# whcorkran/mamba-TTS-project

Hardware: AMD Instinct MI355X
Metric: audio tokens/sec (teacher-forced fwd+bwd) per GPU; decode_step p50 latency (higher is better)
Workload: dtype bf16; 1 GPU; C2: MambaTTSDecoder 12L d_model=1024 fwd+bwd+clip+Adam, B=8/GPU T_audio=2048 T_text=128; model=MambaTTSDecoder-12L-d1024, global_batch=8, seq_len=2048, parallelism=dp1

## Files before the change

### mamba-tts-project_amd/mtts/csrc/skinny.hip

```cpp
#include "common.h"

namespace mtts {
namespace {

typedef short s16x8 __attribute__((ext_vector_type(8)));
typedef __bf16 bf16x8 __attribute__((ext_vector_type(8)));
typedef float f32x4 __attribute__((ext_vector_type(4)));

__device__ __forceinline__ f32x4 mfma16(const uint4& x, const uint4& y, f32x4 c) {
  return __builtin_amdgcn_mfma_f32_16x16x32_bf16(__builtin_bit_cast(bf16x8, x), __builtin_bit_cast(bf16x8, y), c, 0, 0,
                                                 0);
}

struct SkinnyP {
  const bf16_t* a;
  const bf16_t* b;
  void* c;
  int64_t lda, ldb, ldc;
  int m, n, k;
  int c_f32;
  float beta;
};

__device__ __forceinline__ void store4(const SkinnyP& p, int row, int col, f32x4 v) {
  if (row >= p.m || col >= p.n) return;
  if (p.c_f32) {
    float* cp = (float*)p.c + (int64_t)row * p.ldc + col;
    if (p.beta != 0.f) v += p.beta * *(const f32x4*)cp;
    *(f32x4*)cp = v;
  } else {
    bf16_t* cp = (bf16_t*)p.c + (int64_t)row * p.ldc + col;
    if (p.beta != 0.f) {
      const uint2 o = *(const uint2*)cp;
      v[0] += p.beta * __uint_as_float(o.x << 16);
      v[1] += p.beta * __uint_as_float(o.x & 0xffff0000u);
      v[2] += p.beta * __uint_as_float(o.y << 16);
      v[3] += p.beta * __uint_as_float(o.y & 0xffff0000u);
    }
    *(uint2*)cp = make_uint2((uint32_t)f2bf(v[0]) | ((uint32_t)f2bf(v[1]) << 16),
                             (uint32_t)f2bf(v[2]) | ((uint32_t)f2bf(v[3]) << 16));
  }
}

template <int MB, int NB>
__global__ __launch_bounds__(256) void skinny_n_kernel(SkinnyP p) {
  constexpr int RB = MB * 16;
  constexpr int PA = 4;
  __shared__ __attribute__((aligned(16))) f32x4 red[2][MB * NB][64];
  const int lane = threadIdx.x & 63, wave = threadIdx.x >> 6;
  const int row0 = blockIdx.x * RB;
  const int li = lane & 15, kq = (lane >> 4) * 8;
  const bf16_t* ap[MB];
  const bf16_t* bp[NB];
#pragma unroll
  for (int i = 0; i < MB; ++i) ap[i] = p.a + (int64_t)min(row0 + i * 16 + li, p.m - 1) * p.lda + kq + wave * 32;
#pragma unroll
  for (int j = 0; j < NB; ++j) bp[j] = p.b + (int64_t)min(j * 16 + li, p.n - 1) * p.ldb + kq + wave * 32;
  f32x4 acc[MB][NB];
#pragma unroll
  for (int i = 0; i < MB; ++i)
#pragma unroll
    for (int j = 0; j < NB; ++j) acc[i][j] = f32x4{0.f, 0.f, 0.f, 0.f};
  const int ni = (p.k / 32 - wave + 3) / 4;
  uint4 fa[PA][MB], fb[2][NB];
  auto load_a = [&](int i, int st) __attribute__((always_inline)) {
#pragma unroll
    for (int r = 0; r < MB; ++r) fa[st][r] = *(const uint4*)(ap[r] + i * 128);
  };
  auto load_b = [&](int i, int st) __attribute__((always_inline)) {
#pragma unroll
    for (int j = 0; j < NB; ++j) fb[st][j] = *(const uint4*)(bp[j] + i * 128);
  };
#pragma unroll
  for (int j = 0; j < PA; ++j)
    if (j < ni) load_a(j, j);
  if (ni > 0) load_b(0, 0);
  for (int i0 = 0; i0 < ni; i0 += PA) {
#pragma unroll
    for (int j = 0; j < PA; ++j) {
      const int i = i0 + j;
      if (i < ni) {
        if (i + 1 < ni) load_b(i + 1, (j + 1) & 1);
#pragma unroll
        for (int r = 0; r < MB; ++r)
#pragma unroll
          for (int c = 0; c < NB; ++c) acc[r][c] = mfma16(fb[j & 1][c], fa[j][r], acc[r][c]);
        if (i + PA < ni) load_a(i + PA, j);
      }
    }
  }
  if (wave >= 2) {
#pragma unroll
    for (int i = 0; i < MB; ++i)
#pragma unroll
      for (int j = 0; j < NB; ++j) red[wave - 2][i * NB + j][lane] = acc[i][j];
  }
  block_sync();
  if (wave < 2) {
#pragma unroll
    for (int i = 0; i < MB; ++i)
#pragma unroll
      for (int j = 0; j < NB; ++j) acc[i][j] += red[wave][i * NB + j][lane];
  }
  block_sync();
  if (wave == 1) {
#pragma unroll
    for (int i = 0; i < MB; ++i)
#pragma unroll
      for (int j = 0; j < NB; ++j) red[0][i * NB + j][lane] = acc[i][j];
  }
  block_sync();
  if (wave == 0) {
#pragma unroll
    for (int i = 0; i < MB; ++i)
#pragma unroll
      for (int j = 0; j < NB; ++j) store4(p, row0 + i * 16 + li, j * 16 + (lane >> 4) * 4, acc[i][j] + red[0][i * NB + j][lane]);
  }
}

template <int KS>
__global__ __launch_bounds__(256) void small_k_kernel(SkinnyP p) {
  const int lane = threadIdx.x & 63, wave = threadIdx.x >> 6;
  const int row0 = blockIdx.y * 64;
  const int col0 = blockIdx.x * 256 + wave * 64;
  if (col0 >= p.n) return;
  const int li = lane & 15, kq = (lane >> 4) * 8;
  const int g = lane >> 4;
  const int cw_off = (g & 1) * 16 + 8 * (g >> 1);
  uint4 old16[4][2];
  f32x4 old32[4][4];
  if (p.beta != 0.f) {
#pragma unroll
    for (int i = 0; i < 4; ++i) {
      const int row = row0 + i * 16 + li;
      if (p.c_f32) {
#pragma unroll
        for (int j = 0; j < 4; ++j) {
          const int col = col0 + j * 16 + 4 * g;
          old32[i][j] = (row < p.m && col < p.n) ? *(const f32x4*)((const float*)p.c + (int64_t)row * p.ldc + col)
                                                 : f32x4{0.f, 0.f, 0.f, 0.f};
        }
      } else {
#pragma unroll
        for (int q = 0; q < 2; ++q) {
          const int cw = col0 + q * 32 + cw_off;
          old16[i][q] = (row < p.m && cw < p.n) ? *(const uint4*)((const bf16_t*)p.c + (int64_t)row * p.ldc + cw)
                                                : make_uint4(0, 0, 0, 0);
        }
      }
    }
  }
  uint4 fa[4][KS], fb[4][KS];
#pragma unroll
  for (int i = 0; i < 4; ++i) {
    const bf16_t* ap = p.a + (int64_t)min(row0 + i * 16 + li, p.m - 1) * p.lda + kq;
#pragma unroll
    for (int s = 0; s < KS; ++s) fa[i][s] = *(const uint4*)(ap + s * 32);
  }
#pragma unroll
  for (int j = 0; j < 4; ++j) {
    const bf16_t* bp = p.b + (int64_t)min(col0 + j * 16 + li, p.n - 1) * p.ldb + kq;
#pragma unroll
    for (int s = 0; s < KS; ++s) fb[j][s] = *(const uint4*)(bp + s * 32);
  }
  f32x4 acc[4][4];
#pragma unroll
  for (int i = 0; i < 4; ++i)
#pragma unroll
    for (int j = 0; j < 4; ++j) {
      acc[i][j] = f32x4{0.f, 0.f, 0.f, 0.f};
#pragma unroll
      for (int s = 0; s < KS; ++s) acc[i][j] = mfma16(fb[j][s], fa[i][s], acc[i][j]);
    }
  if (p.c_f32) {
#pragma unroll
    for (int i = 0; i < 4; ++i) {
      const int row = row0 + i * 16 + li;
#pragma unroll
      for (int j = 0; j < 4; ++j) {
        const int col = col0 + j * 16 + 4 * g;
        f32x4 v = acc[i][j];
        if (p.beta != 0.f) v += p.beta * old32[i][j];
        if (row < p.m && col < p.n) *(f32x4*)((float*)p.c + (int64_t)row * p.ldc + col) = v;
      }
    }
    return;
  }
#pragma unroll
  for (int i = 0; i < 4; ++i) {
    const int row = row0 + i * 16 + li;
#pragma unroll
    for (int q = 0; q < 2; ++q) {
      float v8[8];
#pragma unroll
      for (int e = 0; e < 4; ++e) {
        const auto r = __builtin_amdgcn_permlane16_swap(__float_as_uint(acc[i][2 * q][e]),
                                                        __float_as_uint(acc[i][2 * q + 1][e]), false, false);
        v8[e] = __uint_as_float(r[0]);
        v8[4 + e] = __uint_as_float(r[1]);
      }
      if (p.beta != 0.f) {
        const uint32_t ow[4] = {old16[i][q].x, old16[i][q].y, old16[i][q].z, old16[i][q].w};
#pragma unroll
        for (int e = 0; e < 4; ++e) {
          v8[2 * e] += p.beta * __uint_as_float(ow[e] << 16);
          v8[2 * e + 1] += p.beta * __uint_as_float(ow[e] & 0xffff0000u);
        }
      }
      uint32_t w[4];
#pragma unroll
      for (int e = 0; e < 4; ++e) w[e] = (uint32_t)f2bf(v8[2 * e]) | ((uint32_t)f2bf(v8[2 * e + 1]) << 16);
      const int cw = col0 + q * 32 + cw_off;
      if (row < p.m && cw < p.n) *(uint4*)((bf16_t*)p.c + (int64_t)row * p.ldc + cw) = make_uint4(w[0], w[1], w[2], w[3]);
    }
  }
}

constexpr int kTnRows = 64;
__device__ __forceinline__ int tn_off(int row, int ch) {
  return 256 * row + 16 * (ch ^ (((row & 3) << 2) | ((row >> 2) & 3)));
}
typedef short s16x4 __attribute__((ext_vector_type(4)));
typedef __attribute__((address_space(3))) s16x4 lds_s16x4;
__device__ __forceinline__ uint4 tn_frag(const char* img, int cb, int ks, int lane) {
  const int g = lane >> 4, q = (lane >> 2) & 3, pp = lane & 3;
  s16x4 r[2];
#pragma unroll
  for (int h = 0; h < 2; ++h) {
    const int row = ks * 32 + 8 * g + 4 * h + q;
    const int off = tn_off(row, cb * 2 + (pp >> 1)) + 8 * (pp & 1);
    r[h] = __builtin_amdgcn_ds_read_tr16_b64_v4i16((lds_s16x4*)(img + off));
  }
  s16x8 v{r[0][0], r[0][1], r[0][2], r[0][3], r[1][0], r[1][1], r[1][2], r[1][3]};
  return __builtin_bit_cast(uint4, v);
}

struct TnP {
  const bf16_t* a;
  const bf16_t* b;
  float* slab;
  int64_t lda, ldb;
  int m, n, k, kc;
};

template <int NB, bool TRANS>
__global__ __launch_bounds__(512) void tn_skinny_kernel(TnP p) {
  __shared__ __attribute__((aligned(16))) char sa[2][kTnRows * 256];
  __shared__ __attribute__((aligned(16))) char sb[2][kTnRows * 256];
  const int tid = threadIdx.x, lane = tid & 63, wave = tid >> 6;
  const int c0 = blockIdx.x * 128;
  const int k0 = blockIdx.y * p.kc, k1 = min(p.k, k0 + p.kc);
  const int ntile = (k1 - k0 + kTnRows - 1) / kTnRows;
  const int ch = tid & 15, r0 = tid >> 4;
  const bool bok = ch * 8 < p.n;
  uint4 ra[2], rb[2];
  auto load = [&](int t) __attribute__((always_inline)) {
#pragma unroll
    for (int s = 0; s < 2; ++s) {
      const int row = k0 + t * kTnRows + r0 + 32 * s;
      const bool ok = row < k1;
      const int rr = ok ? row : k0;
      ra[s] = *(const uint4*)(p.a + (int64_t)rr * p.lda + c0 + ch * 8);
      rb[s] = *(const uint4*)(p.b + (int64_t)rr * p.ldb + (bok ? ch * 8 : 0));
      if (!ok) ra[s] = make_uint4(0, 0, 0, 0);
      if (!ok || !bok) rb[s] = make_uint4(0, 0, 0, 0);
    }
  };
  auto store = [&](int buf) __attribute__((always_inline)) {
#pragma unroll
    for (int s = 0; s < 2; ++s) {
      *(uint4*)(sa[buf] + tn_off(r0 + 32 * s, ch)) = ra[s];
      *(uint4*)(sb[buf] + tn_off(r0 + 32 * s, ch)) = rb[s];
    }
  };
  f32x4 acc[NB];
#pragma unroll
  for (int j = 0; j < NB; ++j) acc[j] = f32x4{0.f, 0.f, 0.f, 0.f};
  if (ntile > 0) {
    load(0);
    store(0);
  }
  block_sync();
  for (int t = 0; t < ntile; ++t) {
    const int buf = t & 1;
    if (t + 1 < ntile) load(t + 1);
#pragma unroll
    for (int ks = 0; ks < 2; ++ks) {
      const uint4 fa = tn_frag(sa[buf], wave, ks, lane);
#pragma unroll
      for (int j = 0; j < NB; ++j) {
        const uint4 fb = tn_frag(sb[buf], j, ks, lane);
        acc[j] = TRANS ? mfma16(fa, fb, acc[j]) : mfma16(fb, fa, acc[j]);
      }
    }
    if (t + 1 < ntile) store(buf ^ 1);
    block_sync();
  }
  float* sl = p.slab + (int64_t)blockIdx.y * p.m * p.n;
  const int li = lane & 15, g4 = (lane >> 4) * 4;
#pragma unroll
  for (int j = 0; j < NB; ++j) {
    if constexpr (TRANS) {
      const int nn = j * 16 + li;
      if (nn < p.n) *(f32x4*)(sl + (int64_t)nn * p.m + c0 + wave * 16 + g4) = acc[j];
    } else {
      const int nn = j * 16 + g4;
      if (nn < p.n) *(f32x4*)(sl + (int64_t)(c0 + wave * 16 + li) * p.n + nn) = acc[j];
    }
  }
}

template <int MB>
void launch_skinny_n(const SkinnyP& p, hipStream_t st) {
  const int nb = (p.n + 15) / 16;
  const dim3 grid((p.m + MB * 16 - 1) / (MB * 16));
  switch (nb) {
#define SK_(N) case N: hipLaunchKernelGGL((skinny_n_kernel<MB, N>), grid, dim3(256), 0, st, p); break;
    SK_(1) SK_(2) SK_(3) SK_(4) SK_(5) SK_(6) SK_(7) SK_(8)
#undef SK_
  }
}

}
}

using namespace mtts;

static int tn_chunk(int k) { return k >= 8192 ? 512 : 256; }

extern "C" int64_t mtts_gemm_skinny_workspace(const MttsSkinnyArgs* a) {
  if (!a || a->mode != MTTS_SKINNY_TN || a->k <= 0) return 0;
  const int kc = tn_chunk(a->k);
  return (int64_t)((a->k + kc - 1) / kc) * a->m * a->n * 4 + 256;
}

static int skinny_tn(const MttsSkinnyArgs* a, hipStream_t st) {
  MTTS_CHECK(a->m % 128 == 0 && a->n <= 128 && a->n % 8 == 0,
             "gemm_skinny TN: needs m %% 128 == 0 and n <= 128, n %% 8 == 0 (m=%d n=%d)", a->m, a->n);
  MTTS_CHECK(a->c_dtype == MTTS_F32 && a->beta == 0.f, "gemm_skinny TN: fp32 output, beta = 0");
  MTTS_CHECK(a->workspace, "gemm_skinny TN: workspace required (mtts_gemm_skinny_workspace)");
  MTTS_CHECK(a->ldc == (a->trans_c ? a->m : a->n), "gemm_skinny TN: C must be contiguous (ldc = %d)",
             a->trans_c ? a->m : a->n);
  MTTS_CHECK(a->lda >= a->m && a->ldb >= a->n, "gemm_skinny TN: leading dimension too small");
  TnP p;
  p.a = (const bf16_t*)a->a; p.b = (const bf16_t*)a->b; p.slab = (float*)a->workspace;
  p.lda = a->lda; p.ldb = a->ldb; p.m = a->m; p.n = a->n; p.k = a->k; p.kc = tn_chunk(a->k);
  const int chunks = (a->k + p.kc - 1) / p.kc;
  const dim3 grid(a->m / 128, chunks);
  const int nb = (a->n + 15) / 16;
#define TN_(N)                                                                                        \
  case N:                                                                                             \
    if (a->trans_c) hipLaunchKernelGGL((tn_skinny_kernel<N, true>), grid, dim3(512), 0, st, p);      \
    else hipLaunchKernelGGL((tn_skinny_kernel<N, false>), grid, dim3(512), 0, st, p);                \
    break;
  switch (nb) { TN_(1) TN_(2) TN_(3) TN_(4) TN_(5) TN_(6) TN_(7) TN_(8) }
#undef TN_
  MTTS_LAUNCH_CHECK("gemm_skinny TN");
  const int ncols = a->m * a->n;
  colsum(p.slab, chunks, chunks, ncols, ncols, (float*)a->c, 0, st);
  MTTS_LAUNCH_CHECK("gemm_skinny TN chunk sum");
  return MTTS_OK;
}

extern "C" int mtts_gemm_skinny(const MttsSkinnyArgs* a, void* stream) {
  MTTS_CHECK(a && a->a && a->b && a->c, "gemm_skinny: null pointer");
  MTTS_CHECK(a->mode == MTTS_SKINNY_N || a->mode == MTTS_SKINNY_SMALL_K || a->mode == MTTS_SKINNY_TN,
             "gemm_skinny: bad mode %d", a->mode);
  MTTS_CHECK(a->m > 0 && a->n > 0 && a->k > 0, "gemm_skinny: m=%d n=%d k=%d must be positive", a->m, a->n, a->k);
  if (a->mode == MTTS_SKINNY_TN) {
    MTTS_CHECK(((uintptr_t)a->a | (uintptr_t)a->b | (uintptr_t)a->c) % 16 == 0 && a->lda % 8 == 0 && a->ldb % 8 == 0,
               "gemm_skinny TN: A / B / C must be 16-byte aligned with row strides a multiple of 8 elements");
    return skinny_tn(a, (hipStream_t)stream);
  }
  MTTS_CHECK(a->k % 32 == 0, "gemm_skinny: k=%d must be a multiple of 32", a->k);
  MTTS_CHECK(a->n % 4 == 0, "gemm_skinny: n=%d must be a multiple of 4", a->n);
  MTTS_CHECK(a->mode != MTTS_SKINNY_N || a->n <= 128, "gemm_skinny: SKINNY_N needs n <= 128 (n=%d)", a->n);
  MTTS_CHECK(a->mode != MTTS_SKINNY_SMALL_K || a->k <= 128, "gemm_skinny: SMALL_K needs k <= 128 (k=%d)", a->k);
  MTTS_CHECK(((uintptr_t)a->a | (uintptr_t)a->b) % 16 == 0 && a->lda % 8 == 0 && a->ldb % 8 == 0,
             "gemm_skinny: A / B must be 16-byte aligned with row strides a multiple of 8 elements");
  MTTS_CHECK(a->lda >= a->k && a->ldb >= a->k && a->ldc >= a->n, "gemm_skinny: leading dimension too small");
  MTTS_CHECK(a->c_dtype == MTTS_F32 || a->c_dtype == MTTS_BF16, "gemm_skinny: bad c_dtype");
  const int ces = a->c_dtype == MTTS_F32 ? 4 : 2;
  MTTS_CHECK((uintptr_t)a->c % (4 * ces) == 0 && a->ldc % 4 == 0,
             "gemm_skinny: C must be %d-byte aligned with ldc a multiple of 4", 4 * ces);
  MTTS_CHECK(a->mode != MTTS_SKINNY_SMALL_K || ces == 4 ||
                 (a->n % 8 == 0 && a->ldc % 8 == 0 && (uintptr_t)a->c % 16 == 0),
             "gemm_skinny: SMALL_K with bf16 C needs n %% 8 == 0, ldc %% 8 == 0 and a 16-byte aligned C "
             "(n=%d ldc=%d)", a->n, a->ldc);
  SkinnyP p;
  p.a = (const bf16_t*)a->a; p.b = (const bf16_t*)a->b; p.c = a->c;
  p.lda = a->lda; p.ldb = a->ldb; p.ldc = a->ldc;
  p.m = a->m; p.n = a->n; p.k = a->k;
  p.c_f32 = a->c_dtype == MTTS_F32;
  p.beta = a->beta;
  hipStream_t st = (hipStream_t)stream;
  if (a->mode == MTTS_SKINNY_N) {
    launch_skinny_n<4>(p, st);
  } else {
    const dim3 grid((a->n + 255) / 256, (a->m + 63) / 64);
    switch (a->k / 32) {
      case 1: hipLaunchKernelGGL((small_k_kernel<1>), grid, dim3(256), 0, st, p); break;
      case 2: hipLaunchKernelGGL((small_k_kernel<2>), grid, dim3(256), 0, st, p); break;
      case 3: hipLaunchKernelGGL((small_k_kernel<3>), grid, dim3(256), 0, st, p); break;
      default: hipLaunchKernelGGL((small_k_kernel<4>), grid, dim3(256), 0, st, p); break;
    }
  }
  MTTS_LAUNCH_CHECK("gemm_skinny");
  return MTTS_OK;
}
```

Baseline: 515,300 tokens/s.

## Restructure skinny GEMM kernels to stage tiles through swizzled LDS

The skinny-N kernel changes from per-wave K-splitting with an LDS reduction to one where each wave owns 16 rows. A and B tiles are cooperatively loaded into a double-buffered, XOR-swizzled LDS ring with register prefetch, and the output goes through LDS staging so stores are coalesced row-wise. The small-K kernel now stages A in LDS once per block instead of every wave reloading it from global memory. It also transposes accumulators through LDS for coalesced stores and sets a launch-bounds occupancy hint. This removes the cross-wave reduction and the redundant global loads, at the cost of a block barrier per K-tile and extra LDS traffic.

```diff
diff --git a/mamba-tts-project_amd/mtts/csrc/skinny.hip b/mamba-tts-project_amd/mtts/csrc/skinny.hip
--- a/mamba-tts-project_amd/mtts/csrc/skinny.hip
+++ b/mamba-tts-project_amd/mtts/csrc/skinny.hip
@@ -22,8 +22,7 @@
   float beta;
 };
 
-__device__ __forceinline__ void store4(const SkinnyP& p, int row, int col, f32x4 v) {
-  if (row >= p.m || col >= p.n) return;
+__device__ __forceinline__ void store_piece4(const SkinnyP& p, int row, int col, f32x4 v) {
   if (p.c_f32) {
     float* cp = (float*)p.c + (int64_t)row * p.ldc + col;
     if (p.beta != 0.f) v += p.beta * *(const f32x4*)cp;
@@ -42,177 +41,190 @@
   }
 }
 
-template <int MB, int NB>
-__global__ __launch_bounds__(256) void skinny_n_kernel(SkinnyP p) {
-  constexpr int RB = MB * 16;
-  constexpr int PA = 4;
-  __shared__ __attribute__((aligned(16))) f32x4 red[2][MB * NB][64];
-  const int lane = threadIdx.x & 63, wave = threadIdx.x >> 6;
-  const int row0 = blockIdx.x * RB;
-  const int li = lane & 15, kq = (lane >> 4) * 8;
-  const bf16_t* ap[MB];
-  const bf16_t* bp[NB];
-#pragma unroll
-  for (int i = 0; i < MB; ++i) ap[i] = p.a + (int64_t)min(row0 + i * 16 + li, p.m - 1) * p.lda + kq + wave * 32;
-#pragma unroll
-  for (int j = 0; j < NB; ++j) bp[j] = p.b + (int64_t)min(j * 16 + li, p.n - 1) * p.ldb + kq + wave * 32;
-  f32x4 acc[MB][NB];
-#pragma unroll
-  for (int i = 0; i < MB; ++i)
-#pragma unroll
-    for (int j = 0; j < NB; ++j) acc[i][j] = f32x4{0.f, 0.f, 0.f, 0.f};
-  const int ni = (p.k / 32 - wave + 3) / 4;
-  uint4 fa[PA][MB], fb[2][NB];
-  auto load_a = [&](int i, int st) __attribute__((always_inline)) {
-#pragma unroll
-    for (int r = 0; r < MB; ++r) fa[st][r] = *(const uint4*)(ap[r] + i * 128);
+__device__ __forceinline__ int kt_off(int row, int ch) { return row * 128 + ((ch ^ ((row >> 1) & 7)) << 4); }
+
+constexpr int kSkPF = 4;
+static_assert(kSkPF % 2 == 0, "kSkPF must be even");
+constexpr int kSkNW = 4;
+constexpr int kSkRB = 16 * kSkNW;
+constexpr int kSkRP = 8 * kSkNW;
+
+template <int NB>
+__global__ __launch_bounds__(64 * kSkNW) void skinny_n_kernel(SkinnyP p) {
+  constexpr int WR = NB * 16;
+  constexpr int WCH = (WR + kSkRP - 1) / kSkRP;
+  constexpr int A_BYTES = kSkRB * 128, SLOT = A_BYTES + WR * 128;
+  constexpr int CP = WR + 4;
+  static_assert(2 * SLOT >= kSkNW * 16 * CP * 4, "C staging fits the ring");
+  __shared__ __attribute__((aligned(16))) char lds[2 * SLOT];
+  const int tid = threadIdx.x, lane = tid & 63, wave = tid >> 6;
+  const int row0 = blockIdx.x * kSkRB;
+  const int ch = tid & 7, lr = (tid >> 3) & (kSkRP - 1);
+  const int li = lane & 15, g = lane >> 4;
+  const bf16_t* ap[2];
+  const bf16_t* bp[WCH];
+#pragma unroll
+  for (int s = 0; s < 2; ++s) ap[s] = p.a + (int64_t)min(row0 + lr + kSkRP * s, p.m - 1) * p.lda + ch * 8;
+#pragma unroll
+  for (int i = 0; i < WCH; ++i) bp[i] = p.b + (int64_t)min(lr + kSkRP * i, p.n - 1) * p.ldb + ch * 8;
+  f32x4 acc[NB];
+#pragma unroll
+  for (int j = 0; j < NB; ++j) acc[j] = f32x4{0.f, 0.f, 0.f, 0.f};
+  const int nt = (p.k + 63) / 64;
+  uint4 ra[kSkPF][2], rb[kSkPF][WCH];
+  auto load = [&](int t, int st) __attribute__((always_inline)) {
+    t = min(t, nt - 1);
+    const int ko = t * 64 - (t * 64 + ch * 8 < p.k ? 0 : 32);
+#pragma unroll
+    for (int s = 0; s < 2; ++s) ra[st][s] = *(const uint4*)(ap[s] + ko);
+#pragma unroll
+    for (int i = 0; i < WCH; ++i) rb[st][i] = *(const uint4*)(bp[i] + ko);
   };
-  auto load_b = [&](int i, int st) __attribute__((always_inline)) {
-#pragma unroll
-    for (int j = 0; j < NB; ++j) fb[st][j] = *(const uint4*)(bp[j] + i * 128);
+  auto stash = [&](int t, int st, int slot) __attribute__((always_inline)) {
+    char* sa = lds + slot * SLOT;
+    const uint32_t km = t * 64 + ch * 8 < p.k ? 0xffffffffu : 0u;
+    auto keep = [&](const uint4& v) { return make_uint4(v.x & km, v.y & km, v.z & km, v.w & km); };
+#pragma unroll
+    for (int s = 0; s < 2; ++s) *(uint4*)(sa + kt_off(lr + kSkRP * s, ch)) = keep(ra[st][s]);
+#pragma unroll
+    for (int i = 0; i < WCH; ++i)
+      if (lr + kSkRP * i < WR) *(uint4*)(sa + A_BYTES + kt_off(lr + kSkRP * i, ch)) = keep(rb[st][i]);
   };
-#pragma unroll
-  for (int j = 0; j < PA; ++j)
-    if (j < ni) load_a(j, j);
-  if (ni > 0) load_b(0, 0);
-  for (int i0 = 0; i0 < ni; i0 += PA) {
-#pragma unroll
-    for (int j = 0; j < PA; ++j) {
-      const int i = i0 + j;
-      if (i < ni) {
-        if (i + 1 < ni) load_b(i + 1, (j + 1) & 1);
-#pragma unroll
-        for (int r = 0; r < MB; ++r)
-#pragma unroll
-          for (int c = 0; c < NB; ++c) acc[r][c] = mfma16(fb[j & 1][c], fa[j][r], acc[r][c]);
-        if (i + PA < ni) load_a(i + PA, j);
+  auto compute = [&](int slot) __attribute__((always_inline)) {
+    const char* sa = lds + slot * SLOT;
+#pragma unroll
+    for (int s = 0; s < 2; ++s) {
+      const uint4 fa = *(const uint4*)(sa + kt_off(16 * wave + li, 4 * s + g));
+#pragma unroll
+      for (int j = 0; j < NB; ++j) {
+        const uint4 fb = *(const uint4*)(sa + A_BYTES + kt_off(16 * j + li, 4 * s + g));
+        acc[j] = mfma16(fb, fa, acc[j]);
       }
     }
-  }
-  if (wave >= 2) {
-#pragma unroll
-    for (int i = 0; i < MB; ++i)
-#pragma unroll
-      for (int j = 0; j < NB; ++j) red[wave - 2][i * NB + j][lane] = acc[i][j];
+  };
+#pragma unroll
+  for (int j = 0; j < kSkPF; ++j) load(j, j);
+  const int tl = (nt - 1) / kSkPF * kSkPF;
+  for (int t0 = 0; t0 < tl; t0 += kSkPF) {
+#pragma unroll
+    for (int j = 0; j < kSkPF; ++j) {
+      stash(t0 + j, j, j & 1);
+      load(t0 + j + kSkPF, j);
+      block_sync();
+      compute(j & 1);
+    }
+  }
+#pragma unroll
+  for (int j = 0; j < kSkPF; ++j) {
+    if (tl + j < nt) {
+      stash(tl + j, j, j & 1);
+      block_sync();
+      compute(j & 1);
+    }
   }
   block_sync();
-  if (wave < 2) {
-#pragma unroll
-    for (int i = 0; i < MB; ++i)
-#pragma unroll
-      for (int j = 0; j < NB; ++j) acc[i][j] += red[wave][i * NB + j][lane];
-  }
+  float* ct = (float*)lds + wave * 16 * CP;
+#pragma unroll
+  for (int j = 0; j < NB; ++j) *(f32x4*)(ct + li * CP + 16 * j + 4 * g) = acc[j];
+  __builtin_amdgcn_s_waitcnt(0xC07F);
+  __builtin_amdgcn_wave_barrier();
+  const int un = p.n >> 2;
+  for (int idx = lane; idx < 16 * un; idx += 64) {
+    const int r = idx / un, x = idx - r * un;
+    const int row = row0 + 16 * wave + r;
+    if (row < p.m) store_piece4(p, row, 4 * x, *(const f32x4*)(ct + r * CP + 4 * x));
+  }
+}
+
+template <int KS>
+__global__ __launch_bounds__(256, 2) void small_k_kernel(SkinnyP p) {
+  constexpr int CPR = 4 * KS;
+  constexpr int AP = (CPR + 1) * 16;
+  __shared__ __attribute__((aligned(16))) char sa[64 * AP];
+  __shared__ __attribute__((aligned(16))) float stg[4][16 * 64];
+  const int tid = threadIdx.x, lane = tid & 63, wave = tid >> 6;
+  const int col0 = blockIdx.x * 256 + wave * 64;
+  const bool active = col0 < p.n;
+  const int li = lane & 15, g = lane >> 4;
+  const int row0 = blockIdx.y * 64;
+  const int r16 = lane >> 3, c16 = col0 + 8 * (lane & 7);
+  const int r32 = lane >> 4, c32 = col0 + 4 * (lane & 15);
+  uint4 fb[4][KS];
+#pragma unroll
+  for (int j = 0; j < 4; ++j) {
+    const bf16_t* bp = p.b + (int64_t)min(col0 + j * 16 + li, p.n - 1) * p.ldb + g * 8;
+#pragma unroll
+    for (int s = 0; s < KS; ++s) fb[j][s] = *(const uint4*)(bp + s * 32);
+  }
+#pragma unroll
+  for (int i = 0; i < KS; ++i) {
+    const int c = tid + 256 * i;
+    *(uint4*)(sa + (c / CPR) * AP + (c % CPR) * 16) =
+        *(const uint4*)(p.a + (int64_t)min(row0 + c / CPR, p.m - 1) * p.lda + (c % CPR) * 8);
+  }
+  float* t = stg[wave];
+  auto unit = [&](int r, int x) __attribute__((always_inline)) { return t + r * 64 + ((x ^ (r & 7)) << 2); };
   block_sync();
-  if (wave == 1) {
-#pragma unroll
-    for (int i = 0; i < MB; ++i)
-#pragma unroll
-      for (int j = 0; j < NB; ++j) red[0][i * NB + j][lane] = acc[i][j];
-  }
-  block_sync();
-  if (wave == 0) {
-#pragma unroll
-    for (int i = 0; i < MB; ++i)
-#pragma unroll
-      for (int j = 0; j < NB; ++j) store4(p, row0 + i * 16 + li, j * 16 + (lane >> 4) * 4, acc[i][j] + red[0][i * NB + j][lane]);
-  }
-}
-
-template <int KS>
-__global__ __launch_bounds__(256) void small_k_kernel(SkinnyP p) {
-  const int lane = threadIdx.x & 63, wave = threadIdx.x >> 6;
-  const int row0 = blockIdx.y * 64;
-  const int col0 = blockIdx.x * 256 + wave * 64;
-  if (col0 >= p.n) return;
-  const int li = lane & 15, kq = (lane >> 4) * 8;
-  const int g = lane >> 4;
-  const int cw_off = (g & 1) * 16 + 8 * (g >> 1);
+  if (!active) return;
   uint4 old16[4][2];
-  f32x4 old32[4][4];
-  if (p.beta != 0.f) {
-#pragma unroll
-    for (int i = 0; i < 4; ++i) {
-      const int row = row0 + i * 16 + li;
-      if (p.c_f32) {
-#pragma unroll
-        for (int j = 0; j < 4; ++j) {
-          const int col = col0 + j * 16 + 4 * g;
-          old32[i][j] = (row < p.m && col < p.n) ? *(const f32x4*)((const float*)p.c + (int64_t)row * p.ldc + col)
-                                                 : f32x4{0.f, 0.f, 0.f, 0.f};
-        }
-      } else {
-#pragma unroll
-        for (int q = 0; q < 2; ++q) {
-          const int cw = col0 + q * 32 + cw_off;
-          old16[i][q] = (row < p.m && cw < p.n) ? *(const uint4*)((const bf16_t*)p.c + (int64_t)row * p.ldc + cw)
-                                                : make_uint4(0, 0, 0, 0);
+  if (p.beta != 0.f && !p.c_f32) {
+#pragma unroll
+    for (int i = 0; i < 4; ++i)
+#pragma unroll
+      for (int h = 0; h < 2; ++h) {
+        const int row = row0 + i * 16 + 8 * h + r16;
+        old16[i][h] = (row < p.m && c16 < p.n) ? *(const uint4*)((const bf16_t*)p.c + (int64_t)row * p.ldc + c16)
+                                               : make_uint4(0, 0, 0, 0);
+      }
+  }
+#pragma unroll
+  for (int i = 0; i < 4; ++i) {
+    uint4 fa[KS];
+#pragma unroll
+    for (int s = 0; s < KS; ++s) fa[s] = *(const uint4*)(sa + (i * 16 + li) * AP + (4 * s + g) * 16);
+    f32x4 acc[4];
+#pragma unroll
+    for (int j = 0; j < 4; ++j) {
+      acc[j] = f32x4{0.f, 0.f, 0.f, 0.f};
+#pragma unroll
+      for (int s = 0; s < KS; ++s) acc[j] = mfma16(fb[j][s], fa[s], acc[j]);
+    }
+#pragma unroll
+    for (int j = 0; j < 4; ++j) *(f32x4*)unit(li, 4 * j + g) = acc[j];
+    __builtin_amdgcn_s_waitcnt(0xC07F);
+    __builtin_amdgcn_wave_barrier();
+    if (p.c_f32) {
+#pragma unroll
+      for (int h = 0; h < 4; ++h) {
+        const int r = 4 * h + r32, row = row0 + i * 16 + r;
+        f32x4 v = *(const f32x4*)unit(r, lane & 15);
+        if (row < p.m && c32 < p.n) {
+          float* cp = (float*)p.c + (int64_t)row * p.ldc + c32;
+          if (p.beta != 0.f) v += p.beta * *(const f32x4*)cp;
+          *(f32x4*)cp = v;
         }
       }
-    }
-  }
-  uint4 fa[4][KS], fb[4][KS];
-#pragma unroll
-  for (int i = 0; i < 4; ++i) {
-    const bf16_t* ap = p.a + (int64_t)min(row0 + i * 16 + li, p.m - 1) * p.lda + kq;
-#pragma unroll
-    for (int s = 0; s < KS; ++s) fa[i][s] = *(const uint4*)(ap + s * 32);
-  }
-#pragma unroll
-  for (int j = 0; j < 4; ++j) {
-    const bf16_t* bp = p.b + (int64_t)min(col0 + j * 16 + li, p.n - 1) * p.ldb + kq;
-#pragma unroll
-    for (int s = 0; s < KS; ++s) fb[j][s] = *(const uint4*)(bp + s * 32);
-  }
-  f32x4 acc[4][4];
-#pragma unroll
-  for (int i = 0; i < 4; ++i)
-#pragma unroll
-    for (int j = 0; j < 4; ++j) {
-      acc[i][j] = f32x4{0.f, 0.f, 0.f, 0.f};
-#pragma unroll
-      for (int s = 0; s < KS; ++s) acc[i][j] = mfma16(fb[j][s], fa[i][s], acc[i][j]);
-    }
-  if (p.c_f32) {
-#pragma unroll
-    for (int i = 0; i < 4; ++i) {
-      const int row = row0 + i * 16 + li;
-#pragma unroll
-      for (int j = 0; j < 4; ++j) {
-        const int col = col0 + j * 16 + 4 * g;
-        f32x4 v = acc[i][j];
-        if (p.beta != 0.f) v += p.beta * old32[i][j];
-        if (row < p.m && col < p.n) *(f32x4*)((float*)p.c + (int64_t)row * p.ldc + col) = v;
+    } else {
+#pragma unroll
+      for (int h = 0; h < 2; ++h) {
+        const int r = 8 * h + r16, row = row0 + i * 16 + r;
+        const f32x4 lo = *(const f32x4*)unit(r, 2 * (lane & 7)), hi = *(const f32x4*)unit(r, 2 * (lane & 7) + 1);
+        float v8[8] = {lo[0], lo[1], lo[2], lo[3], hi[0], hi[1], hi[2], hi[3]};
+        if (p.beta != 0.f) {
+          const uint32_t ow[4] = {old16[i][h].x, old16[i][h].y, old16[i][h].z, old16[i][h].w};
+#pragma unroll
+          for (int e = 0; e < 4; ++e) {
+            v8[2 * e] += p.beta * __uint_as_float(ow[e] << 16);
+            v8[2 * e + 1] += p.beta * __uint_as_float(ow[e] & 0xffff0000u);
+          }
+        }
+        uint32_t w[4];
+#pragma unroll
+        for (int e = 0; e < 4; ++e) w[e] = (uint32_t)f2bf(v8[2 * e]) | ((uint32_t)f2bf(v8[2 * e + 1]) << 16);
+        if (row < p.m && c16 < p.n) *(uint4*)((bf16_t*)p.c + (int64_t)row * p.ldc + c16) = make_uint4(w[0], w[1], w[2], w[3]);
       }
     }
-    return;
-  }
-#pragma unroll
-  for (int i = 0; i < 4; ++i) {
-    const int row = row0 + i * 16 + li;
-#pragma unroll
-    for (int q = 0; q < 2; ++q) {
-      float v8[8];
-#pragma unroll
-      for (int e = 0; e < 4; ++e) {
-        const auto r = __builtin_amdgcn_permlane16_swap(__float_as_uint(acc[i][2 * q][e]),
-                                                        __float_as_uint(acc[i][2 * q + 1][e]), false, false);
-        v8[e] = __uint_as_float(r[0]);
-        v8[4 + e] = __uint_as_float(r[1]);
-      }
-      if (p.beta != 0.f) {
-        const uint32_t ow[4] = {old16[i][q].x, old16[i][q].y, old16[i][q].z, old16[i][q].w};
-#pragma unroll
-        for (int e = 0; e < 4; ++e) {
-          v8[2 * e] += p.beta * __uint_as_float(ow[e] << 16);
-          v8[2 * e + 1] += p.beta * __uint_as_float(ow[e] & 0xffff0000u);
-        }
-      }
-      uint32_t w[4];
-#pragma unroll
-      for (int e = 0; e < 4; ++e) w[e] = (uint32_t)f2bf(v8[2 * e]) | ((uint32_t)f2bf(v8[2 * e + 1]) << 16);
-      const int cw = col0 + q * 32 + cw_off;
-      if (row < p.m && cw < p.n) *(uint4*)((bf16_t*)p.c + (int64_t)row * p.ldc + cw) = make_uint4(w[0], w[1], w[2], w[3]);
-    }
+    __builtin_amdgcn_wave_barrier();
   }
 }
 
@@ -310,12 +322,11 @@
   }
 }
 
-template <int MB>
 void launch_skinny_n(const SkinnyP& p, hipStream_t st) {
   const int nb = (p.n + 15) / 16;
-  const dim3 grid((p.m + MB * 16 - 1) / (MB * 16));
+  const dim3 grid((p.m + kSkRB - 1) / kSkRB);
   switch (nb) {
-#define SK_(N) case N: hipLaunchKernelGGL((skinny_n_kernel<MB, N>), grid, dim3(256), 0, st, p); break;
+#define SK_(N) case N: hipLaunchKernelGGL((skinny_n_kernel<N>), grid, dim3(64 * kSkNW), 0, st, p); break;
     SK_(1) SK_(2) SK_(3) SK_(4) SK_(5) SK_(6) SK_(7) SK_(8)
 #undef SK_
   }
@@ -395,7 +406,7 @@
   p.beta = a->beta;
   hipStream_t st = (hipStream_t)stream;
   if (a->mode == MTTS_SKINNY_N) {
-    launch_skinny_n<4>(p, st);
+    launch_skinny_n(p, st);
   } else {
     const dim3 grid((a->n + 255) / 256, (a->m + 63) / 64);
     switch (a->k / 32) {
```

New measurement: 520,000 tokens/s, median of 6. Within noise of the previous version (+0.9%).
